# EthanD11/RS-VIO

Measured on AMD Instinct MI355X. Metric: stereo frames/sec (tracker+BA) on 752×480 EuRoC stream; BA ms/iter at window=10, higher is better.
Workload: dtype f32 (tracker) / f64 (BA)

## Files before the change

### rs-vio_amd/csrc/pyramid.hip

```cpp
#include "pyramid.hpp"

namespace rsvio {

namespace {

constexpr int TW = 64;
constexpr int TH = 8;
constexpr int STRIP_COLS = 320;
constexpr size_t LDS_CAP = 64 << 10;

__device__ __forceinline__ float triangle_kernel(float x) {
    float ax = fabsf(x);
    return ax < 1.0f ? 1.0f - ax : 0.0f;
}

__global__ void make_taps_kernel(TapTable tab, int n_entries) {
    int e = blockIdx.x * blockDim.x + threadIdx.x;
    if (e >= n_entries) return;
    int in_len = tab.ent_in_len[e];
    int out_len = tab.ent_out_len[e];
    int o = tab.ent_out_idx[e];
    float ratio = (float)in_len / (float)out_len;
    float sratio = ratio < 1.0f ? 1.0f : ratio;
    float support = 1.0f * sratio;
    float inputc = ((float)o + 0.5f) * ratio;
    long long left = (long long)floorf(inputc - support);
    if (left < 0) left = 0;
    if (left > (long long)in_len - 1) left = in_len - 1;
    long long right = (long long)ceilf(inputc + support);
    if (right < left + 1) right = left + 1;
    if (right > (long long)in_len) right = in_len;
    inputc = inputc - 0.5f;
    int cnt = (int)(right - left);
    float* w = tab.weights + (size_t)e * tab.max_taps;
    float sum = 0.0f;
    for (int k = 0; k < cnt; ++k) {
        float wv = triangle_kernel(((float)(left + k) - inputc) / sratio);
        w[k] = wv;
        sum += wv;
    }
    for (int k = 0; k < cnt; ++k) w[k] = w[k] / sum;
    tab.left[e] = (int)left;
    tab.count[e] = cnt;
}

__global__ __launch_bounds__(256) void pyramid_kernel(PyrLaunch L, PyrIO io) {
    extern __shared__ uint32_t smem[];
    const int img = blockIdx.y;
    {
        const int fb = (int)blockIdx.x - (L.copy_blocks + L.tile_start[L.levels]);
        if (fb >= 0) {
            if (io.table != nullptr) {
                const PyrSlot d = io.table[img];
                if (d.fast_pt != nullptr && fb < io.fast_cells)
                    fast_cell(d.src, io.fg, fb, nullptr, nullptr, 0, d.fast_pt, d.fast_aff,
                              reinterpret_cast<uint8_t*>(smem));
            } else if (img == 0 && fb < io.fast_cells) {
                const uint8_t* s0 = io.psrc ? io.psrc : io.src[0];
                fast_cell(s0, io.fg, fb, nullptr, nullptr, 0, io.fast_pt, io.fast_aff,
                          reinterpret_cast<uint8_t*>(smem));
            }
            return;
        }
    }
    const uint8_t* __restrict__ src =
        io.table ? io.table[img].src : (io.psrc ? io.psrc + (size_t)img * L.w * L.h : io.src[img]);
    uint8_t* __restrict__ dst_base =
        io.table ? io.table[img].dst : (io.psrc ? io.pdst + (size_t)img * L.pyr_bytes : io.dst[img]);
    int b = blockIdx.x;
    const bool aligned = ((reinterpret_cast<uintptr_t>(src) | reinterpret_cast<uintptr_t>(dst_base)) & 15) == 0;
    if (b < L.copy_blocks) {
        const size_t tot = (size_t)L.w * L.h;
        if (!aligned) {
            for (size_t i = (size_t)b * blockDim.x + threadIdx.x; i < tot; i += (size_t)L.copy_blocks * blockDim.x)
                dst_base[i] = src[i];
            return;
        }
        const size_t n16 = tot / 16;
        const uint4* s4 = reinterpret_cast<const uint4*>(src);
        uint4* d4 = reinterpret_cast<uint4*>(dst_base);
        for (size_t i = (size_t)b * blockDim.x + threadIdx.x; i < n16; i += (size_t)L.copy_blocks * blockDim.x)
            d4[i] = s4[i];
        size_t tail0 = n16 * 16;
        if (b == 0)
            for (size_t i = tail0 + threadIdx.x; i < tot; i += blockDim.x) dst_base[i] = src[i];
        return;
    }
    b -= L.copy_blocks;
    int lev = 1;
    while (lev < L.levels - 1 && b >= L.tile_start[lev + 1]) ++lev;
    b -= L.tile_start[lev];
    const int nw = (int)level_w(L.w, lev), nh = (int)level_h(L.h, lev);
    const int tw = L.tile_w[lev], th = L.tile_h[lev];
    const int tiles_x = (nw + tw - 1) / tw;
    const int tx = b % tiles_x, ty = b / tiles_x;
    const int ox0 = tx * tw, ox1 = min(ox0 + tw, nw);
    const int oy0 = ty * th, oy1 = min(oy0 + th, nh);
    const int rows = oy1 - oy0, cols_out = ox1 - ox0;
    const int hx = L.hx_ent[lev], vy = L.vy_ent[lev];
    const TapTable& T = L.tab;
    const int xl = T.left[hx + ox0];
    const int xr = T.left[hx + ox1 - 1] + T.count[hx + ox1 - 1];
    const int yl = T.left[vy + oy0];
    const int yr = T.left[vy + oy1 - 1] + T.count[vy + oy1 - 1];
    const int ncols = xr - xl, nrows = yr - yl;
    const int xa = xl & ~3, xoff = xl - xa;
    const int pd = (xr - xa + 3) >> 2;
    const bool direct = (L.direct >> lev) & 1;
    uint8_t* strip = reinterpret_cast<uint8_t*>(smem);
    if (!direct) {
        if (aligned && (L.w & 3) == 0) {
            const uint32_t* s32 = reinterpret_cast<const uint32_t*>(src);
            const int wd = (int)(L.w >> 2);
            for (int idx = threadIdx.x; idx < nrows * pd; idx += blockDim.x) {
                const int r = idx / pd, d = idx - r * pd;
                smem[idx] = s32[(size_t)(yl + r) * wd + (xa >> 2) + d];
            }
        } else {
            for (int idx = threadIdx.x; idx < nrows * pd * 4; idx += blockDim.x) {
                const int r = idx / (pd * 4), c = idx - r * pd * 4;
                strip[idx] = (xa + c < (int)L.w) ? src[(size_t)(yl + r) * L.w + xa + c] : 0;
            }
        }
    }
    float* tmp = reinterpret_cast<float*>(smem + (direct ? 0 : nrows * pd));
    __syncthreads();
    for (int idx = threadIdx.x; idx < rows * ncols; idx += blockDim.x) {
        const int r = idx / ncols, c = idx - r * ncols;
        const int e = vy + oy0 + r;
        const int vl = T.left[e], vc = T.count[e];
        const float* __restrict__ vw = T.weights + (size_t)e * T.max_taps;
        float acc = 0.0f;
        if (!direct) {
            const uint8_t* col = strip + (vl - yl) * pd * 4 + xoff + c;
            for (int k = 0; k < vc; ++k) acc += (float)col[k * pd * 4] * vw[k];
        } else {
            const uint8_t* __restrict__ col = src + (size_t)vl * L.w + xl + c;
            for (int k = 0; k < vc; k += 8) {
                float px[8];
#pragma unroll
                for (int u = 0; u < 8; ++u) px[u] = (k + u < vc) ? (float)col[(size_t)(k + u) * L.w] : 0.0f;
#pragma unroll
                for (int u = 0; u < 8; ++u)
                    if (k + u < vc) acc += px[u] * vw[k + u];
            }
        }
        tmp[r * ncols + c] = acc;
    }
    __syncthreads();
    uint8_t* __restrict__ dst = dst_base + level_offset(L.w, L.h, lev);
    for (int idx = threadIdx.x; idx < rows * cols_out; idx += blockDim.x) {
        const int r = idx / cols_out, c = idx - r * cols_out;
        const int e = hx + ox0 + c;
        const int hl = T.left[e] - xl, hc = T.count[e];
        const float* __restrict__ hw = T.weights + (size_t)e * T.max_taps;
        const float* __restrict__ row = tmp + r * ncols + hl;
        float acc = 0.0f;
        for (int k = 0; k < hc; ++k) acc += row[k] * hw[k];
        float cl = acc < 0.0f ? 0.0f : (acc > 255.0f ? 255.0f : acc);
        dst[(size_t)(oy0 + r) * nw + ox0 + c] = (uint8_t)roundf(cl);
    }
}

}

void PyramidPlan::init(int w_, int h_, int levels_) {
    w = w_;
    h = h_;
    levels = levels_;
    if (levels < 1 || levels > kMaxLevels) throw std::invalid_argument("levels must be in [1, 8]");
    if (w < 16 || h < 16) throw std::invalid_argument("image too small");
    std::vector<int> in_len, out_len, out_idx;
    float max_ratio = 1.0f;
    memset(&launch, 0, sizeof(launch));
    for (int i = 1; i < levels; ++i) {
        int nw = (int)level_w(w, i), nh = (int)level_h(h, i);
        if (nw < 1 || nh < 1) throw std::invalid_argument("too many levels for image size");
        launch.hx_ent[i] = (int)in_len.size();
        for (int o = 0; o < nw; ++o) { in_len.push_back(w); out_len.push_back(nw); out_idx.push_back(o); }
        launch.vy_ent[i] = (int)in_len.size();
        for (int o = 0; o < nh; ++o) { in_len.push_back(h); out_len.push_back(nh); out_idx.push_back(o); }
        float rx = (float)w / nw, ry = (float)h / nh;
        max_ratio = std::max(max_ratio, std::max(rx, ry));
        launch.tile_h[i] = std::max(1, std::min(TH, (int)(16.0f / ry)));
        launch.tile_w[i] = std::max(1, std::min(TW, (int)std::floor((STRIP_COLS - 2.0f * rx - 4.0f) / rx)));
    }
    n_entries = (int)in_len.size();
    max_taps = (int)std::ceil(2.0f * max_ratio) + 4;
    int tiles = 0;
    for (int i = 1; i < levels; ++i) {
        launch.tile_start[i] = tiles;
        int nw = (int)level_w(w, i), nh = (int)level_h(h, i);
        tiles += ((nw + launch.tile_w[i] - 1) / launch.tile_w[i]) * ((nh + launch.tile_h[i] - 1) / launch.tile_h[i]);
    }
    launch.tile_start[levels] = tiles;
    launch.copy_blocks = std::max(1, (int)(((size_t)w * h / 16 + 255) / 256 / 4));
    total_blocks = launch.copy_blocks + tiles;
    launch.w = (uint32_t)w;
    launch.h = (uint32_t)h;
    launch.levels = levels;
    launch.pyr_bytes = level_offset(w, h, levels);
    if (n_entries > 0) {
        i_in.alloc(n_entries); i_out.alloc(n_entries); i_idx.alloc(n_entries);
        d_left.alloc(n_entries); d_count.alloc(n_entries);
        d_w.alloc((size_t)n_entries * max_taps);
        RSVIO_HIP(hipMemcpy(i_in.p, in_len.data(), sizeof(int) * n_entries, hipMemcpyHostToDevice));
        RSVIO_HIP(hipMemcpy(i_out.p, out_len.data(), sizeof(int) * n_entries, hipMemcpyHostToDevice));
        RSVIO_HIP(hipMemcpy(i_idx.p, out_idx.data(), sizeof(int) * n_entries, hipMemcpyHostToDevice));
        TapTable t;
        t.left = d_left.p; t.count = d_count.p; t.weights = d_w.p; t.max_taps = max_taps;
        t.ent_in_len = i_in.p; t.ent_out_len = i_out.p; t.ent_out_idx = i_idx.p;
        hipLaunchKernelGGL(make_taps_kernel, dim3((n_entries + 255) / 256), dim3(256), 0, 0, t, n_entries);
        RSVIO_HIP(hipGetLastError());
        RSVIO_HIP(hipDeviceSynchronize());
        launch.tab = t;
        std::vector<int> left(n_entries), count(n_entries);
        RSVIO_HIP(hipMemcpy(left.data(), d_left.p, sizeof(int) * n_entries, hipMemcpyDeviceToHost));
        RSVIO_HIP(hipMemcpy(count.data(), d_count.p, sizeof(int) * n_entries, hipMemcpyDeviceToHost));
        for (int i = 1; i < levels; ++i) {
            const int nw = (int)level_w(w, i), nh = (int)level_h(h, i);
            const int tw = launch.tile_w[i], th = launch.tile_h[i];
            size_t strip = 0, vert = 0;
            for (int ox0 = 0; ox0 < nw; ox0 += tw) {
                const int ox1 = std::min(ox0 + tw, nw);
                const int xl = left[launch.hx_ent[i] + ox0];
                const int xr = left[launch.hx_ent[i] + ox1 - 1] + count[launch.hx_ent[i] + ox1 - 1];
                const size_t pd = (size_t)(xr - (xl & ~3) + 3) / 4;
                for (int oy0 = 0; oy0 < nh; oy0 += th) {
                    const int oy1 = std::min(oy0 + th, nh);
                    const int yl = left[launch.vy_ent[i] + oy0];
                    const int yr = left[launch.vy_ent[i] + oy1 - 1] + count[launch.vy_ent[i] + oy1 - 1];
                    strip = std::max(strip, 4 * pd * (size_t)(yr - yl));
                    vert = std::max(vert, 4 * (size_t)(oy1 - oy0) * (size_t)(xr - xl));
                }
            }
            if (vert > LDS_CAP) throw std::invalid_argument("image too wide for the pyramid tile");
            if (strip + vert > LDS_CAP) launch.direct |= 1u << i;
            lds_bytes = std::max(lds_bytes, ((launch.direct >> i) & 1) ? vert : strip + vert);
        }
    }
}

void PyramidPlan::enqueue(const PyrIO& io, int n_img, hipStream_t s) const {
    if (n_img <= 0) return;
    if (n_img > (io.psrc || io.table ? 65535 : kMaxPyrIO)) throw std::invalid_argument("too many images per pyramid launch");
    const size_t lds = io.fast_cells > 0 ? std::max(lds_bytes, (size_t)io.fg.g * io.fg.g) : lds_bytes;
    hipLaunchKernelGGL(pyramid_kernel, dim3(total_blocks + std::max(io.fast_cells, 0), n_img), dim3(256), lds, s,
                       launch, io);
    RSVIO_HIP(hipGetLastError());
}

void PyramidPlan::enqueue(const uint8_t* d_imgs, int n_img, uint8_t* d_pyrs, hipStream_t s) const {
    for (int i0 = 0; i0 < n_img; i0 += 65535) {
        PyrIO io{};
        io.psrc = d_imgs + (size_t)i0 * w * h;
        io.pdst = d_pyrs + (size_t)i0 * pyr_bytes();
        enqueue(io, std::min(65535, n_img - i0), s);
    }
}

}
```

### rs-vio_amd/csrc/pyramid.hpp

```cpp
#pragma once
#include <algorithm>
#include <cmath>
#include <cstring>
#include <stdexcept>
#include <vector>

#include "common.hpp"
#include "fast.hpp"

namespace rsvio {

constexpr int kMaxLevels = 8;

struct TapTable {
    int* left = nullptr;
    int* count = nullptr;
    float* weights = nullptr;
    int max_taps = 0;
    const int* ent_in_len = nullptr;
    const int* ent_out_len = nullptr;
    const int* ent_out_idx = nullptr;
};

struct PyrLaunch {
    uint32_t w, h;
    int levels;
    size_t pyr_bytes;
    int copy_blocks;
    int tile_start[kMaxLevels + 1];
    int tile_w[kMaxLevels];
    int tile_h[kMaxLevels];
    uint32_t direct;
    int hx_ent[kMaxLevels];
    int vy_ent[kMaxLevels];
    TapTable tab;
};

constexpr int kMaxPyrIO = 8;
struct PyrSlot {
    const uint8_t* src;
    uint8_t* dst;
    int4* fast_pt;
    float* fast_aff;
};
struct PyrIO {
    const uint8_t* src[kMaxPyrIO];
    uint8_t* dst[kMaxPyrIO];
    const uint8_t* psrc;
    uint8_t* pdst;
    int fast_cells;
    GridGeom fg;
    int4* fast_pt;
    float* fast_aff;
    const PyrSlot* table;
};

struct PyramidPlan {
    int w = 0, h = 0, levels = 0;
    int n_entries = 0, max_taps = 0, total_blocks = 0;
    size_t lds_bytes = 0;
    PyrLaunch launch;
    DevBuf<int> i_in, i_out, i_idx, d_left, d_count;
    DevBuf<float> d_w;
    void init(int w, int h, int levels);
    size_t pyr_bytes() const { return level_offset(w, h, levels); }
    void enqueue(const uint8_t* d_imgs, int n_img, uint8_t* d_pyrs, hipStream_t s) const;
    void enqueue(const PyrIO& io, int n_img, hipStream_t s) const;
};

}
```

Before: 5101.

## Precompute per-tile pyramid descriptors and stage interleaved tap records in LDS

Moves per-block tile geometry into a host-built 64-byte tile table, so blocks no longer search levels or divide to find their tile. Tap left/count/weights are packed into per-entry interleaved records that each block prefetches into LDS alongside the source strip. The vertical pass now handles four packed bytes per dword thread and writes float4, and index math uses shifts instead of divides. The copy path is unrolled with batched 16-byte loads. Tile sizes grow (16 rows, 128 columns, 256-column strip), which raises LDS use per block and may lower occupancy.

Result: no change. 5104, median of 2 (+0.1%).

```diff
diff --git a/rs-vio_amd/csrc/pyramid.hip b/rs-vio_amd/csrc/pyramid.hip
--- a/rs-vio_amd/csrc/pyramid.hip
+++ b/rs-vio_amd/csrc/pyramid.hip
@@ -4,10 +4,9 @@
 
 namespace {
 
-constexpr int TW = 64;
-constexpr int TH = 8;
-constexpr int STRIP_COLS = 320;
-constexpr size_t LDS_CAP = 64 << 10;
+constexpr int kStripPer = 10;
+constexpr int kTapPer = 4;
+typedef uint32_t u32x4 __attribute__((ext_vector_type(4)));
 
 __device__ __forceinline__ float triangle_kernel(float x) {
     float ax = fabsf(x);
@@ -32,7 +31,8 @@
     if (right > (long long)in_len) right = in_len;
     inputc = inputc - 0.5f;
     int cnt = (int)(right - left);
-    float* w = tab.weights + (size_t)e * tab.max_taps;
+    uint32_t* rec = tab.rec + tab.ent_rec_off[e];
+    float* w = reinterpret_cast<float*>(rec + 2);
     float sum = 0.0f;
     for (int k = 0; k < cnt; ++k) {
         float wv = triangle_kernel(((float)(left + k) - inputc) / sratio);
@@ -40,15 +40,16 @@
         sum += wv;
     }
     for (int k = 0; k < cnt; ++k) w[k] = w[k] / sum;
-    tab.left[e] = (int)left;
-    tab.count[e] = cnt;
+    rec[0] = (uint32_t)(int)left;
+    rec[1] = (uint32_t)cnt;
 }
 
 __global__ __launch_bounds__(256) void pyramid_kernel(PyrLaunch L, PyrIO io) {
-    extern __shared__ uint32_t smem[];
+    extern __shared__ __align__(16) uint32_t smem[];
     const int img = blockIdx.y;
+    const int tid = threadIdx.x;
     {
-        const int fb = (int)blockIdx.x - (L.copy_blocks + L.tile_start[L.levels]);
+        const int fb = (int)blockIdx.x - (L.copy_blocks + L.n_tiles);
         if (fb >= 0) {
             if (io.table != nullptr) {
                 const PyrSlot d = io.table[img];
@@ -72,172 +73,179 @@
     if (b < L.copy_blocks) {
         const size_t tot = (size_t)L.w * L.h;
         if (!aligned) {
-            for (size_t i = (size_t)b * blockDim.x + threadIdx.x; i < tot; i += (size_t)L.copy_blocks * blockDim.x)
+            for (size_t i = (size_t)b * blockDim.x + tid; i < tot; i += (size_t)L.copy_blocks * blockDim.x)
                 dst_base[i] = src[i];
             return;
         }
         const size_t n16 = tot / 16;
-        const uint4* s4 = reinterpret_cast<const uint4*>(src);
-        uint4* d4 = reinterpret_cast<uint4*>(dst_base);
-        for (size_t i = (size_t)b * blockDim.x + threadIdx.x; i < n16; i += (size_t)L.copy_blocks * blockDim.x)
-            d4[i] = s4[i];
+        const u32x4* s4 = reinterpret_cast<const u32x4*>(src);
+        u32x4* d4 = reinterpret_cast<u32x4*>(dst_base);
+        const size_t i0 = (size_t)b * (256 * kPyrCopyPer) + tid;
+        u32x4 v[kPyrCopyPer];
+#pragma unroll
+        for (int u = 0; u < kPyrCopyPer; ++u) v[u] = s4[min(i0 + u * 256, n16 - 1)];
+#pragma unroll
+        for (int u = 0; u < kPyrCopyPer; ++u)
+            if (i0 + u * 256 < n16) d4[i0 + u * 256] = v[u];
         size_t tail0 = n16 * 16;
         if (b == 0)
-            for (size_t i = tail0 + threadIdx.x; i < tot; i += blockDim.x) dst_base[i] = src[i];
+            for (size_t i = tail0 + tid; i < tot; i += blockDim.x) dst_base[i] = src[i];
         return;
     }
     b -= L.copy_blocks;
-    int lev = 1;
-    while (lev < L.levels - 1 && b >= L.tile_start[lev + 1]) ++lev;
-    b -= L.tile_start[lev];
-    const int nw = (int)level_w(L.w, lev), nh = (int)level_h(L.h, lev);
-    const int tw = L.tile_w[lev], th = L.tile_h[lev];
-    const int tiles_x = (nw + tw - 1) / tw;
-    const int tx = b % tiles_x, ty = b / tiles_x;
-    const int ox0 = tx * tw, ox1 = min(ox0 + tw, nw);
-    const int oy0 = ty * th, oy1 = min(oy0 + th, nh);
-    const int rows = oy1 - oy0, cols_out = ox1 - ox0;
-    const int hx = L.hx_ent[lev], vy = L.vy_ent[lev];
-    const TapTable& T = L.tab;
-    const int xl = T.left[hx + ox0];
-    const int xr = T.left[hx + ox1 - 1] + T.count[hx + ox1 - 1];
-    const int yl = T.left[vy + oy0];
-    const int yr = T.left[vy + oy1 - 1] + T.count[vy + oy1 - 1];
-    const int ncols = xr - xl, nrows = yr - yl;
-    const int xa = xl & ~3, xoff = xl - xa;
-    const int pd = (xr - xa + 3) >> 2;
-    const bool direct = (L.direct >> lev) & 1;
-    uint8_t* strip = reinterpret_cast<uint8_t*>(smem);
+    const PyrTile t = L.tiles[b];
+    const int lev = t.lev, rows = t.rows, cols_out = t.cols, rs = t.rs;
+    const int xl = t.xl, yl = t.yl, ncols = t.xr - t.xl, nrows = t.yr - t.yl;
+    const bool direct = t.direct != 0;
+    const PyrTileLds lay = pyr_tile_lds(cols_out, rows, t.xl, t.xr, t.yl, t.yr, rs, t.direct);
+    const int pd = lay.pd, ts = lay.ts;
+    const int xa = xl & ~3;
+    float* tmp = reinterpret_cast<float*>(smem);
+    uint32_t* strip32 = smem + lay.strip_off;
+    uint32_t* vtab = smem + lay.taps_off;
+    const uint32_t* htab = vtab + rows * rs;
+    const int vs = t.vshift, vmask = (1 << vs) - 1;
+    const int vn = rows * rs, tn = vn + cols_out * rs;
+    const uint32_t* __restrict__ vsrc = L.rec + t.vrec;
+    const uint32_t* __restrict__ hsrc = L.rec + t.hrec;
+    const bool by_dword = aligned && (L.w & 3) == 0;
+    {
+        uint32_t tv[kTapPer];
+#pragma unroll
+        for (int u = 0; u < kTapPer; ++u) {
+            const int j = min(tid + u * 256, tn - 1);
+            tv[u] = j < vn ? vsrc[j] : hsrc[j - vn];
+        }
+        if (!direct && by_dword) {
+            const uint32_t* __restrict__ s32 = reinterpret_cast<const uint32_t*>(src) + (size_t)yl * (L.w >> 2) + (xa >> 2);
+            const int wd = (int)(L.w >> 2);
+            const int nidx = nrows << vs;
+            uint32_t sv[kStripPer];
+#pragma unroll
+            for (int u = 0; u < kStripPer; ++u) {
+                const int idx = tid + u * 256, r = min(idx >> vs, nrows - 1), d = min(idx & vmask, pd - 1);
+                sv[u] = s32[(size_t)r * wd + d];
+            }
+#pragma unroll
+            for (int u = 0; u < kStripPer; ++u) {
+                const int idx = tid + u * 256, r = idx >> vs, d = idx & vmask;
+                if (idx < nidx && d < pd) strip32[r * pd + d] = sv[u];
+            }
+            for (int idx = tid + kStripPer * 256; idx < nidx; idx += 256) {
+                const int r = idx >> vs, d = idx & vmask;
+                if (d < pd) strip32[r * pd + d] = s32[(size_t)r * wd + d];
+            }
+        }
+#pragma unroll
+        for (int u = 0; u < kTapPer; ++u) {
+            const int j = tid + u * 256;
+            if (j < tn) vtab[j] = tv[u];
+        }
+        for (int j = tid + kTapPer * 256; j < tn; j += 256) vtab[j] = j < vn ? vsrc[j] : hsrc[j - vn];
+    }
+    if (!direct && !by_dword) {
+        uint8_t* strip = reinterpret_cast<uint8_t*>(strip32);
+        const int bs = vs + 2, bmask = (1 << bs) - 1, pb = pd * 4;
+        for (int idx = tid; idx < (nrows << bs); idx += 256) {
+            const int r = idx >> bs, c = idx & bmask;
+            if (c < pb) strip[r * pb + c] = (xa + c < (int)L.w) ? src[(size_t)(yl + r) * L.w + xa + c] : 0;
+        }
+    }
+    __syncthreads();
     if (!direct) {
-        if (aligned && (L.w & 3) == 0) {
-            const uint32_t* s32 = reinterpret_cast<const uint32_t*>(src);
-            const int wd = (int)(L.w >> 2);
-            for (int idx = threadIdx.x; idx < nrows * pd; idx += blockDim.x) {
-                const int r = idx / pd, d = idx - r * pd;
-                smem[idx] = s32[(size_t)(yl + r) * wd + (xa >> 2) + d];
-            }
-        } else {
-            for (int idx = threadIdx.x; idx < nrows * pd * 4; idx += blockDim.x) {
-                const int r = idx / (pd * 4), c = idx - r * pd * 4;
-                strip[idx] = (xa + c < (int)L.w) ? src[(size_t)(yl + r) * L.w + xa + c] : 0;
-            }
-        }
-    }
-    float* tmp = reinterpret_cast<float*>(smem + (direct ? 0 : nrows * pd));
-    __syncthreads();
-    for (int idx = threadIdx.x; idx < rows * ncols; idx += blockDim.x) {
-        const int r = idx / ncols, c = idx - r * ncols;
-        const int e = vy + oy0 + r;
-        const int vl = T.left[e], vc = T.count[e];
-        const float* __restrict__ vw = T.weights + (size_t)e * T.max_taps;
-        float acc = 0.0f;
-        if (!direct) {
-            const uint8_t* col = strip + (vl - yl) * pd * 4 + xoff + c;
-            for (int k = 0; k < vc; ++k) acc += (float)col[k * pd * 4] * vw[k];
-        } else {
+        for (int idx = tid; idx < (rows << vs); idx += 256) {
+            const int r = idx >> vs, d = idx & vmask;
+            if (d >= pd) continue;
+            const uint32_t* rec = vtab + r * rs;
+            const int vl = (int)rec[0] - yl, vc = (int)rec[1];
+            const uint32_t* col = strip32 + vl * pd + d;
+            float a0 = 0.0f, a1 = 0.0f, a2 = 0.0f, a3 = 0.0f;
+            for (int k = 0; k < vc; ++k) {
+                const uint32_t p = col[k * pd];
+                const float wk = __uint_as_float(rec[2 + k]);
+                a0 += (float)(p & 0xffu) * wk;
+                a1 += (float)((p >> 8) & 0xffu) * wk;
+                a2 += (float)((p >> 16) & 0xffu) * wk;
+                a3 += (float)(p >> 24) * wk;
+            }
+            *reinterpret_cast<float4*>(tmp + r * ts + 4 * d) = make_float4(a0, a1, a2, a3);
+        }
+    } else {
+        for (int idx = tid; idx < rows * ncols; idx += 256) {
+            const int r = idx / ncols, c = idx - r * ncols;
+            const uint32_t* rec = vtab + r * rs;
+            const int vl = (int)rec[0], vc = (int)rec[1];
             const uint8_t* __restrict__ col = src + (size_t)vl * L.w + xl + c;
+            float acc = 0.0f;
             for (int k = 0; k < vc; k += 8) {
                 float px[8];
 #pragma unroll
                 for (int u = 0; u < 8; ++u) px[u] = (k + u < vc) ? (float)col[(size_t)(k + u) * L.w] : 0.0f;
 #pragma unroll
                 for (int u = 0; u < 8; ++u)
-                    if (k + u < vc) acc += px[u] * vw[k + u];
-            }
-        }
-        tmp[r * ncols + c] = acc;
+                    if (k + u < vc) acc += px[u] * __uint_as_float(rec[2 + k + u]);
+            }
+            tmp[r * ts + c] = acc;
+        }
     }
     __syncthreads();
-    uint8_t* __restrict__ dst = dst_base + level_offset(L.w, L.h, lev);
-    for (int idx = threadIdx.x; idx < rows * cols_out; idx += blockDim.x) {
-        const int r = idx / cols_out, c = idx - r * cols_out;
-        const int e = hx + ox0 + c;
-        const int hl = T.left[e] - xl, hc = T.count[e];
-        const float* __restrict__ hw = T.weights + (size_t)e * T.max_taps;
-        const float* __restrict__ row = tmp + r * ncols + hl;
+    const int nw = (int)level_w(L.w, lev);
+    uint8_t* __restrict__ dst = dst_base + level_offset(L.w, L.h, lev) + (size_t)t.oy0 * nw + t.ox0;
+    const int x0 = direct ? xl : xa;
+    const int hs = t.hshift, hmask = (1 << hs) - 1;
+    for (int idx = tid; idx < (rows << hs); idx += 256) {
+        const int r = idx >> hs, c = idx & hmask;
+        if (c >= cols_out) continue;
+        const uint32_t* rec = htab + c * rs;
+        const int hl = (int)rec[0] - x0, hc = (int)rec[1];
+        const float* row = tmp + r * ts + hl;
         float acc = 0.0f;
-        for (int k = 0; k < hc; ++k) acc += row[k] * hw[k];
+        for (int k = 0; k < hc; ++k) acc += row[k] * __uint_as_float(rec[2 + k]);
         float cl = acc < 0.0f ? 0.0f : (acc > 255.0f ? 255.0f : acc);
-        dst[(size_t)(oy0 + r) * nw + ox0 + c] = (uint8_t)roundf(cl);
+        dst[(size_t)r * nw + c] = (uint8_t)roundf(cl);
     }
 }
 
 }
 
 void PyramidPlan::init(int w_, int h_, int levels_) {
+    tiles = pyr_plan_tiles(w_, h_, levels_);
     w = w_;
     h = h_;
     levels = levels_;
-    if (levels < 1 || levels > kMaxLevels) throw std::invalid_argument("levels must be in [1, 8]");
-    if (w < 16 || h < 16) throw std::invalid_argument("image too small");
-    std::vector<int> in_len, out_len, out_idx;
-    float max_ratio = 1.0f;
+    n_entries = tiles.n_entries;
     memset(&launch, 0, sizeof(launch));
-    for (int i = 1; i < levels; ++i) {
-        int nw = (int)level_w(w, i), nh = (int)level_h(h, i);
-        if (nw < 1 || nh < 1) throw std::invalid_argument("too many levels for image size");
-        launch.hx_ent[i] = (int)in_len.size();
-        for (int o = 0; o < nw; ++o) { in_len.push_back(w); out_len.push_back(nw); out_idx.push_back(o); }
-        launch.vy_ent[i] = (int)in_len.size();
-        for (int o = 0; o < nh; ++o) { in_len.push_back(h); out_len.push_back(nh); out_idx.push_back(o); }
-        float rx = (float)w / nw, ry = (float)h / nh;
-        max_ratio = std::max(max_ratio, std::max(rx, ry));
-        launch.tile_h[i] = std::max(1, std::min(TH, (int)(16.0f / ry)));
-        launch.tile_w[i] = std::max(1, std::min(TW, (int)std::floor((STRIP_COLS - 2.0f * rx - 4.0f) / rx)));
-    }
-    n_entries = (int)in_len.size();
-    max_taps = (int)std::ceil(2.0f * max_ratio) + 4;
-    int tiles = 0;
-    for (int i = 1; i < levels; ++i) {
-        launch.tile_start[i] = tiles;
-        int nw = (int)level_w(w, i), nh = (int)level_h(h, i);
-        tiles += ((nw + launch.tile_w[i] - 1) / launch.tile_w[i]) * ((nh + launch.tile_h[i] - 1) / launch.tile_h[i]);
-    }
-    launch.tile_start[levels] = tiles;
-    launch.copy_blocks = std::max(1, (int)(((size_t)w * h / 16 + 255) / 256 / 4));
-    total_blocks = launch.copy_blocks + tiles;
     launch.w = (uint32_t)w;
     launch.h = (uint32_t)h;
     launch.levels = levels;
     launch.pyr_bytes = level_offset(w, h, levels);
+    launch.copy_blocks = tiles.copy_blocks;
+    launch.n_tiles = (int)tiles.tiles.size();
+    total_blocks = launch.copy_blocks + launch.n_tiles;
+    lds_bytes = tiles.lds_bytes;
     if (n_entries > 0) {
-        i_in.alloc(n_entries); i_out.alloc(n_entries); i_idx.alloc(n_entries);
-        d_left.alloc(n_entries); d_count.alloc(n_entries);
-        d_w.alloc((size_t)n_entries * max_taps);
-        RSVIO_HIP(hipMemcpy(i_in.p, in_len.data(), sizeof(int) * n_entries, hipMemcpyHostToDevice));
-        RSVIO_HIP(hipMemcpy(i_out.p, out_len.data(), sizeof(int) * n_entries, hipMemcpyHostToDevice));
-        RSVIO_HIP(hipMemcpy(i_idx.p, out_idx.data(), sizeof(int) * n_entries, hipMemcpyHostToDevice));
+        i_in.alloc(n_entries); i_out.alloc(n_entries); i_idx.alloc(n_entries); i_off.alloc(n_entries);
+        d_rec.alloc(tiles.rec_dwords);
+        d_tiles.alloc(tiles.tiles.size());
+        RSVIO_HIP(hipMemcpy(i_in.p, tiles.in_len.data(), sizeof(int) * n_entries, hipMemcpyHostToDevice));
+        RSVIO_HIP(hipMemcpy(i_out.p, tiles.out_len.data(), sizeof(int) * n_entries, hipMemcpyHostToDevice));
+        RSVIO_HIP(hipMemcpy(i_idx.p, tiles.out_idx.data(), sizeof(int) * n_entries, hipMemcpyHostToDevice));
+        RSVIO_HIP(hipMemcpy(i_off.p, tiles.rec_off.data(), sizeof(int) * n_entries, hipMemcpyHostToDevice));
+        RSVIO_HIP(hipMemcpy(d_tiles.p, tiles.tiles.data(), sizeof(PyrTile) * tiles.tiles.size(), hipMemcpyHostToDevice));
+        RSVIO_HIP(hipMemset(d_rec.p, 0, sizeof(uint32_t) * tiles.rec_dwords));
         TapTable t;
-        t.left = d_left.p; t.count = d_count.p; t.weights = d_w.p; t.max_taps = max_taps;
-        t.ent_in_len = i_in.p; t.ent_out_len = i_out.p; t.ent_out_idx = i_idx.p;
+        t.rec = d_rec.p;
+        t.ent_in_len = i_in.p; t.ent_out_len = i_out.p; t.ent_out_idx = i_idx.p; t.ent_rec_off = i_off.p;
         hipLaunchKernelGGL(make_taps_kernel, dim3((n_entries + 255) / 256), dim3(256), 0, 0, t, n_entries);
         RSVIO_HIP(hipGetLastError());
         RSVIO_HIP(hipDeviceSynchronize());
-        launch.tab = t;
-        std::vector<int> left(n_entries), count(n_entries);
-        RSVIO_HIP(hipMemcpy(left.data(), d_left.p, sizeof(int) * n_entries, hipMemcpyDeviceToHost));
-        RSVIO_HIP(hipMemcpy(count.data(), d_count.p, sizeof(int) * n_entries, hipMemcpyDeviceToHost));
-        for (int i = 1; i < levels; ++i) {
-            const int nw = (int)level_w(w, i), nh = (int)level_h(h, i);
-            const int tw = launch.tile_w[i], th = launch.tile_h[i];
-            size_t strip = 0, vert = 0;
-            for (int ox0 = 0; ox0 < nw; ox0 += tw) {
-                const int ox1 = std::min(ox0 + tw, nw);
-                const int xl = left[launch.hx_ent[i] + ox0];
-                const int xr = left[launch.hx_ent[i] + ox1 - 1] + count[launch.hx_ent[i] + ox1 - 1];
-                const size_t pd = (size_t)(xr - (xl & ~3) + 3) / 4;
-                for (int oy0 = 0; oy0 < nh; oy0 += th) {
-                    const int oy1 = std::min(oy0 + th, nh);
-                    const int yl = left[launch.vy_ent[i] + oy0];
-                    const int yr = left[launch.vy_ent[i] + oy1 - 1] + count[launch.vy_ent[i] + oy1 - 1];
-                    strip = std::max(strip, 4 * pd * (size_t)(yr - yl));
-                    vert = std::max(vert, 4 * (size_t)(oy1 - oy0) * (size_t)(xr - xl));
-                }
-            }
-            if (vert > LDS_CAP) throw std::invalid_argument("image too wide for the pyramid tile");
-            if (strip + vert > LDS_CAP) launch.direct |= 1u << i;
-            lds_bytes = std::max(lds_bytes, ((launch.direct >> i) & 1) ? vert : strip + vert);
-        }
+        launch.tiles = d_tiles.p;
+        launch.rec = d_rec.p;
+        std::vector<uint32_t> rec(tiles.rec_dwords);
+        RSVIO_HIP(hipMemcpy(rec.data(), d_rec.p, sizeof(uint32_t) * rec.size(), hipMemcpyDeviceToHost));
+        for (int e = 0; e < n_entries; ++e)
+            if ((int)rec[tiles.rec_off[e]] != tiles.left[e] || (int)rec[tiles.rec_off[e] + 1] != tiles.count[e])
+                throw std::runtime_error("pyramid tap spans differ between host and device");
     }
 }
 
diff --git a/rs-vio_amd/csrc/pyramid.hpp b/rs-vio_amd/csrc/pyramid.hpp
--- a/rs-vio_amd/csrc/pyramid.hpp
+++ b/rs-vio_amd/csrc/pyramid.hpp
@@ -7,33 +7,26 @@
 
 #include "common.hpp"
 #include "fast.hpp"
+#include "pyramid_tiles.hpp"
 
 namespace rsvio {
 
-constexpr int kMaxLevels = 8;
-
 struct TapTable {
-    int* left = nullptr;
-    int* count = nullptr;
-    float* weights = nullptr;
-    int max_taps = 0;
+    uint32_t* rec = nullptr;
     const int* ent_in_len = nullptr;
     const int* ent_out_len = nullptr;
     const int* ent_out_idx = nullptr;
+    const int* ent_rec_off = nullptr;
 };
 
 struct PyrLaunch {
     uint32_t w, h;
     int levels;
+    int copy_blocks;
+    int n_tiles;
     size_t pyr_bytes;
-    int copy_blocks;
-    int tile_start[kMaxLevels + 1];
-    int tile_w[kMaxLevels];
-    int tile_h[kMaxLevels];
-    uint32_t direct;
-    int hx_ent[kMaxLevels];
-    int vy_ent[kMaxLevels];
-    TapTable tab;
+    const PyrTile* tiles;
+    const uint32_t* rec;
 };
 
 constexpr int kMaxPyrIO = 8;
@@ -57,11 +50,13 @@
 
 struct PyramidPlan {
     int w = 0, h = 0, levels = 0;
-    int n_entries = 0, max_taps = 0, total_blocks = 0;
+    int n_entries = 0, total_blocks = 0;
     size_t lds_bytes = 0;
     PyrLaunch launch;
-    DevBuf<int> i_in, i_out, i_idx, d_left, d_count;
-    DevBuf<float> d_w;
+    PyrTilePlan tiles;
+    DevBuf<int> i_in, i_out, i_idx, i_off;
+    DevBuf<uint32_t> d_rec;
+    DevBuf<PyrTile> d_tiles;
     void init(int w, int h, int levels);
     size_t pyr_bytes() const { return level_offset(w, h, levels); }
     void enqueue(const uint8_t* d_imgs, int n_img, uint8_t* d_pyrs, hipStream_t s) const;
diff --git a/rs-vio_amd/csrc/pyramid_tiles.hpp b/rs-vio_amd/csrc/pyramid_tiles.hpp
--- /dev/null
+++ b/rs-vio_amd/csrc/pyramid_tiles.hpp
@@ -0,0 +1,177 @@
+#pragma once
+#include <algorithm>
+#include <cmath>
+#include <cstddef>
+#include <cstdint>
+#include <stdexcept>
+#include <vector>
+
+namespace rsvio {
+
+constexpr int kMaxLevels = 8;
+constexpr size_t kPyrLdsCap = 64 << 10;
+
+#ifndef RSVIO_PYR_TH
+#define RSVIO_PYR_TH 16
+#endif
+#ifndef RSVIO_PYR_TW
+#define RSVIO_PYR_TW 128
+#endif
+#ifndef RSVIO_PYR_STRIP
+#define RSVIO_PYR_STRIP 256
+#endif
+constexpr int kPyrCopyPer = 4;
+
+struct PyrTile {
+    int lev;
+    int ox0, oy0;
+    int cols, rows;
+    int xl, xr, yl, yr;
+    int vrec, hrec;
+    int rs;
+    int vshift, hshift;
+    int direct;
+    int pad;
+};
+static_assert(sizeof(PyrTile) == 64, "one 64-byte record per tile");
+
+struct PyrTilePlan {
+    int w = 0, h = 0, levels = 0;
+    int tile_w[kMaxLevels] = {}, tile_h[kMaxLevels] = {};
+    int tile_start[kMaxLevels + 1] = {};
+    int hx_ent[kMaxLevels] = {}, vy_ent[kMaxLevels] = {};
+    int rs[kMaxLevels] = {};
+    int n_entries = 0;
+    size_t rec_dwords = 0;
+    uint32_t direct = 0;
+    size_t lds_bytes = 0;
+    int copy_blocks = 0;
+    std::vector<int> in_len, out_len, out_idx;
+    std::vector<int> left, count, rec_off;
+    std::vector<PyrTile> tiles;
+};
+
+inline void pyr_tap_span(int in_len, int out_len, int o, int* left_out, int* count_out) {
+    const float ratio = (float)in_len / (float)out_len;
+    const float sratio = ratio < 1.0f ? 1.0f : ratio;
+    const float support = 1.0f * sratio;
+    const float inputc = ((float)o + 0.5f) * ratio;
+    long long left = (long long)std::floor(inputc - support);
+    if (left < 0) left = 0;
+    if (left > (long long)in_len - 1) left = in_len - 1;
+    long long right = (long long)std::ceil(inputc + support);
+    if (right < left + 1) right = left + 1;
+    if (right > (long long)in_len) right = in_len;
+    *left_out = (int)left;
+    *count_out = (int)(right - left);
+}
+
+inline int pyr_ceil_log2(int n) {
+    int s = 0;
+    while ((1 << s) < n) ++s;
+    return s;
+}
+
+struct PyrTileLds {
+    int pd;
+    int ts;
+    int strip_off;
+    int taps_off;
+    size_t dwords;
+};
+constexpr PyrTileLds pyr_tile_lds(int cols, int rows, int xl, int xr, int yl, int yr, int rs, int direct) {
+    const int pd = (xr - (xl & ~3) + 3) >> 2;
+    const int ts = direct ? xr - xl : 4 * pd;
+    const size_t tmp = (size_t)rows * (size_t)ts;
+    const size_t strip = direct ? 0 : (size_t)(yr - yl) * (size_t)pd;
+    return PyrTileLds{pd, ts, (int)tmp, (int)(tmp + strip), tmp + strip + (size_t)(rows + cols) * (size_t)rs};
+}
+
+inline PyrTilePlan pyr_plan_tiles(int w, int h, int levels) {
+    if (levels < 1 || levels > kMaxLevels) throw std::invalid_argument("levels must be in [1, 8]");
+    if (w < 16 || h < 16) throw std::invalid_argument("image too small");
+    PyrTilePlan P;
+    P.w = w;
+    P.h = h;
+    P.levels = levels;
+    for (int i = 1; i < levels; ++i) {
+        const int nw = w >> i, nh = h >> i;
+        if (nw < 1 || nh < 1) throw std::invalid_argument("too many levels for image size");
+        P.hx_ent[i] = (int)P.in_len.size();
+        for (int o = 0; o < nw; ++o) { P.in_len.push_back(w); P.out_len.push_back(nw); P.out_idx.push_back(o); }
+        P.vy_ent[i] = (int)P.in_len.size();
+        for (int o = 0; o < nh; ++o) { P.in_len.push_back(h); P.out_len.push_back(nh); P.out_idx.push_back(o); }
+        int max_count = 1;
+        for (int e = P.hx_ent[i]; e < (int)P.in_len.size(); ++e) {
+            int l, c;
+            pyr_tap_span(P.in_len[e], P.out_len[e], P.out_idx[e], &l, &c);
+            P.left.push_back(l);
+            P.count.push_back(c);
+            max_count = std::max(max_count, c);
+        }
+        P.rs[i] = 2 + (max_count | 1);
+        for (int e = P.hx_ent[i]; e < (int)P.in_len.size(); ++e) {
+            P.rec_off.push_back((int)P.rec_dwords);
+            P.rec_dwords += (size_t)P.rs[i];
+        }
+        if (P.rec_dwords > (size_t)INT32_MAX) throw std::invalid_argument("image too large for the pyramid tap table");
+        const float rx = (float)w / nw, ry = (float)h / nh;
+        const int th_max = std::max(1, std::min(RSVIO_PYR_TH, (int)(2.0f * RSVIO_PYR_TH / ry)));
+        const int tw_max =
+            std::max(1, std::min(RSVIO_PYR_TW, (int)std::floor((RSVIO_PYR_STRIP - 2.0f * rx - 7.0f) / rx)));
+        const int tiles_x = (nw + tw_max - 1) / tw_max, tiles_y = (nh + th_max - 1) / th_max;
+        P.tile_w[i] = (nw + tiles_x - 1) / tiles_x;
+        P.tile_h[i] = (nh + tiles_y - 1) / tiles_y;
+    }
+    P.n_entries = (int)P.in_len.size();
+    for (int i = 1; i < levels; ++i) {
+        P.tile_start[i] = (int)P.tiles.size();
+        const int nw = w >> i, nh = h >> i;
+        const int tw = P.tile_w[i], th = P.tile_h[i];
+        const size_t first = P.tiles.size();
+        for (int pass = 0; pass < 2; ++pass) {
+            const int direct = (int)((P.direct >> i) & 1);
+            P.tiles.resize(first);
+            size_t level_lds = 0;
+            bool over = false;
+            for (int oy0 = 0; oy0 < nh; oy0 += th)
+                for (int ox0 = 0; ox0 < nw; ox0 += tw) {
+                    const int ox1 = std::min(ox0 + tw, nw), oy1 = std::min(oy0 + th, nh);
+                    const int ex0 = P.hx_ent[i] + ox0, ex1 = P.hx_ent[i] + ox1 - 1;
+                    const int ey0 = P.vy_ent[i] + oy0, ey1 = P.vy_ent[i] + oy1 - 1;
+                    PyrTile t{};
+                    t.lev = i;
+                    t.ox0 = ox0;
+                    t.oy0 = oy0;
+                    t.cols = ox1 - ox0;
+                    t.rows = oy1 - oy0;
+                    t.xl = P.left[ex0];
+                    t.xr = P.left[ex1] + P.count[ex1];
+                    t.yl = P.left[ey0];
+                    t.yr = P.left[ey1] + P.count[ey1];
+                    t.vrec = P.rec_off[ey0];
+                    t.hrec = P.rec_off[ex0];
+                    t.rs = P.rs[i];
+                    t.direct = direct;
+                    const PyrTileLds lds = pyr_tile_lds(t.cols, t.rows, t.xl, t.xr, t.yl, t.yr, t.rs, direct);
+                    t.vshift = pyr_ceil_log2(lds.pd);
+                    t.hshift = pyr_ceil_log2(t.cols);
+                    if (lds.dwords * 4 > kPyrLdsCap) over = true;
+                    level_lds = std::max(level_lds, lds.dwords * 4);
+                    P.tiles.push_back(t);
+                }
+            if (!over) {
+                P.lds_bytes = std::max(P.lds_bytes, level_lds);
+                break;
+            }
+            if (direct) throw std::invalid_argument("image too wide for the pyramid tile");
+            P.direct |= 1u << i;
+        }
+    }
+    P.tile_start[levels] = (int)P.tiles.size();
+    const size_t n16 = (size_t)w * h / 16;
+    P.copy_blocks = std::max<int>(1, (int)((n16 + 256 * kPyrCopyPer - 1) / (256 * kPyrCopyPer)));
+    return P;
+}
+
+}
```
